# dalek-cryptography/curve25519-dalek

Hardware: NVIDIA H100
Metric: Pippenger MSM points/sec (higher is better)
Workload: dtype exact integers: f64 limbs (radix 2^51, FP64 pipe) in the bucket kernel, u32 limbs (radix 2^25.5) elsewhere

## Files before the change

### curve25519_dalek_b200/csrc/msm.cu

```cuda
#include <algorithm>
#include <cstdio>
#include <utility>
#include <vector>

#include "../../include/dalek_b200.h"
#include "engine.h"
#include "ge64.cuh"
#include "warp4.cuh"
#include "warp4_f64.cuh"

static inline unsigned cdiv(size_t a, unsigned b) { return (unsigned)((a + b - 1) / b); }

int ws_reserve(dalek_b200_ctx *ctx, DevBuf &b, size_t bytes)
{
    if (bytes <= b.cap) return 0;
    if (b.p) { cudaFree(b.p); b.p = nullptr; b.cap = 0; }
    size_t want = bytes + bytes / 8 + 256;
    cudaError_t e = cudaMalloc(&b.p, want);
    if (e != cudaSuccess) { ctx->last_error = std::string("cudaMalloc: ") + cudaGetErrorString(e); return DALEK_E_NOMEM; }
    b.cap = want;
    return 0;
}

int pinned_reserve(dalek_b200_ctx *ctx, size_t bytes)
{
    if (bytes <= ctx->h_pinned_cap) return 0;
    if (ctx->h_pinned) cudaFreeHost(ctx->h_pinned);
    ctx->h_pinned = nullptr; ctx->h_pinned_cap = 0;
    cudaError_t e = cudaMallocHost(&ctx->h_pinned, bytes + 4096);
    if (e != cudaSuccess) { ctx->last_error = std::string("cudaMallocHost: ") + cudaGetErrorString(e); return DALEK_E_NOMEM; }
    ctx->h_pinned_cap = bytes + 4096;
    return 0;
}

template <int F64>
__global__ void __launch_bounds__(128, 3) k_prep_compressed(const uint4 *__restrict__ in, ge_niels_packed *__restrict__ out, size_t n,
                                  int *__restrict__ bad)
{
    size_t i = (size_t)blockIdx.x * blockDim.x + threadIdx.x;
    if (i >= n) return;
    uint4 a = in[2 * i], b = in[2 * i + 1];
    uint32_t s[8] = {a.x, a.y, a.z, a.w, b.x, b.y, b.z, b.w};
    fe x, y;
    uint32_t ok = ge_decompress_affine<F64>(x, y, s);
    if (!ok) { atomicOr(bad, 1); fe_0(x); fe_1(y); }
    ge_niels nl; ge_affine_to_niels(nl, x, y);
    ge_niels_packed p; ge_niels_pack(p, nl);
    uint4 *o = reinterpret_cast<uint4 *>(out + i);
#pragma unroll
    for (int k = 0; k < 6; k++) o[k] = make_uint4(p.w[4 * k], p.w[4 * k + 1], p.w[4 * k + 2], p.w[4 * k + 3]);
}

template <int F64>
__global__ void k_prep_ristretto(const uint32_t *__restrict__ in, ge_niels_packed *__restrict__ out, size_t n, int *__restrict__ bad)
{
    size_t i = (size_t)blockIdx.x * blockDim.x + threadIdx.x;
    if (i >= n) return;
    uint32_t enc[8];
#pragma unroll
    for (int k = 0; k < 8; k++) enc[k] = in[8 * i + k];
    ge_p3 P;
    if (!ristretto_decompress<F64>(P, enc)) { atomicOr(bad, 1); ge_p3_identity(P); }
    ge_niels nl; ge_affine_to_niels(nl, P.X, P.Y);
    ge_niels_packed pk; ge_niels_pack(pk, nl);
    out[i] = pk;
}

#define PREP_THREADS 256
#define PREP_PER_THREAD 4
#define PREP_GROUP (PREP_THREADS * PREP_PER_THREAD)
#define PREP_NW (PREP_THREADS / 32)

__device__ __forceinline__ void load_coord_f64(fe64 &h, const uint64_t *__restrict__ src)
{
    uint64_t l[5];
#pragma unroll
    for (int k = 0; k < 5; k++) l[k] = __ldg(src + k);
    fe t; fe_from_limbs51(t, l);
    fe64_from_fe_limbs(h, t);
}
__device__ __forceinline__ void store_coord(uint4 *o, const fe64 &v, uint32_t ok, uint32_t c)
{
    fe f;
    uint32_t w[8];
    fe64_to_fe(f, v); fe_tobytes_words(w, f);
#pragma unroll
    for (int q = 0; q < 8; q++) w[q] = ok ? w[q] : (q == 0 ? c : 0u);
    o[0] = make_uint4(w[0], w[1], w[2], w[3]);
    o[1] = make_uint4(w[4], w[5], w[6], w[7]);
}
__device__ __forceinline__ uint32_t load_z(fe64 &h, const uint64_t *__restrict__ in, size_t i)
{
    uint64_t l[5];
#pragma unroll
    for (int k = 0; k < 5; k++) l[k] = __ldg(in + 20 * i + 10 + k);
    fe t; fe_from_limbs51(t, l);
    fe64_from_fe_limbs(h, t);
    return 1u - (uint32_t)fe_iszero(t);
}
__device__ __forceinline__ void fe64_shfl_up(fe64 &o, const fe64 &f, int d)
{
#pragma unroll
    for (int k = 0; k < 5; k++) o.v[k] = __shfl_up_sync(0xffffffffu, f.v[k], d);
}
__device__ __forceinline__ void fe64_shfl_down(fe64 &o, const fe64 &f, int d)
{
#pragma unroll
    for (int k = 0; k < 5; k++) o.v[k] = __shfl_down_sync(0xffffffffu, f.v[k], d);
}
__device__ __forceinline__ void fe64_shfl_xor(fe64 &o, const fe64 &f, int m)
{
#pragma unroll
    for (int k = 0; k < 5; k++) o.v[k] = __shfl_xor_sync(0xffffffffu, f.v[k], m);
}
__device__ __forceinline__ void fe64_shfl_idx(fe64 &o, const fe64 &f, int src)
{
#pragma unroll
    for (int k = 0; k < 5; k++) o.v[k] = __shfl_sync(0xffffffffu, f.v[k], src);
}

__device__ __forceinline__ void warp_product(fe64 &p, const fe64 &x, int width)
{
    fe64 t;
    p = x;
#pragma unroll 1
    for (int m = width >> 1; m > 0; m >>= 1) { fe64_shfl_xor(t, p, m); fe64_mul(p, p, t); }
}

__device__ __forceinline__ void warp_other_products(const fe64 &x, fe64 &below, fe64 &above, fe64 &all)
{
    const uint32_t lane = threadIdx.x & 31;
    fe64 lo = x, hi = x, t;
#pragma unroll 1
    for (int d = 1; d < 32; d <<= 1) {
        fe64_shfl_up(t, lo, d);
        if (lane >= (uint32_t)d) fe64_mul(lo, lo, t);
        fe64_shfl_down(t, hi, d);
        if (lane + d < 32) fe64_mul(hi, hi, t);
    }
    fe64_shfl_idx(all, lo, 31);
    fe64_shfl_up(below, lo, 1); if (lane == 0) fe64_1(below);
    fe64_shfl_down(above, hi, 1); if (lane == 31) fe64_1(above);
}

template <bool INVERT>
__device__ __forceinline__ void block_inverse(fe64 &inv, const fe64 &acc, fe64 *s_warp, const fe64 *tot_inv)
{
    const uint32_t lane = threadIdx.x & 31, warp = threadIdx.x >> 5, nw = blockDim.x >> 5;
    fe64 below, above, all;
    warp_other_products(acc, below, above, all);
    if (lane == 0) s_warp[warp] = all;
    __syncthreads();
    if (warp == 0) {
        fe64 x, b, a, t;
        if (lane < nw) x = s_warp[lane]; else fe64_1(x);
        warp_other_products(x, b, a, all);
        if (INVERT) {
            fe q; fe64_to_fe(q, all); fe_invert(q, q); fe64_from_fe_limbs(t, q);
        } else {
            t = *tot_inv;
        }
        fe64_mul(t, t, b); fe64_mul(t, t, a);
        if (lane < nw) s_warp[lane] = t;
    }
    __syncthreads();
    fe64_mul(inv, s_warp[warp], below); fe64_mul(inv, inv, above);
}

__global__ void __launch_bounds__(PREP_THREADS, 2)
k_prep_zprod(const uint64_t *__restrict__ in, fe64 *__restrict__ prod, size_t n)
{
    __shared__ fe64 s_warp[PREP_NW];
    const uint32_t tid = threadIdx.x, lane = tid & 31, warp = tid >> 5;
    const size_t g0 = (size_t)blockIdx.x * PREP_GROUP + tid;
    fe64 z[PREP_PER_THREAD], acc, t;
    uint32_t ok[PREP_PER_THREAD];
#pragma unroll
    for (int k = 0; k < PREP_PER_THREAD; k++) {
        const size_t i = g0 + (size_t)k * PREP_THREADS;
        if (i < n) ok[k] = load_z(z[k], in, i); else { ok[k] = 0; fe64_1(z[k]); }
    }
    acc = z[0];
    if (!ok[0]) fe64_1(acc);
#pragma unroll
    for (int k = 1; k < PREP_PER_THREAD; k++) { fe64_mul(t, acc, z[k]); fe64_cmov(acc, t, ok[k]); }
    warp_product(t, acc, 32);
    if (lane == 0) s_warp[warp] = t;
    __syncthreads();
    if (warp == 0) {
        if (lane < PREP_NW) acc = s_warp[lane]; else fe64_1(acc);
        warp_product(t, acc, PREP_NW);
        if (lane == 0) prod[blockIdx.x] = t;
    }
}

__global__ void __launch_bounds__(PREP_THREADS)
k_prep_invert(fe64 *__restrict__ prod, fe64 *__restrict__ pre, uint32_t G)
{
    __shared__ fe64 s_warp[PREP_NW];
    const uint32_t per = (G + blockDim.x - 1) / blockDim.x, b = min(threadIdx.x * per, G), e = min(b + per, G);
    fe64 acc, inv, t;
    fe64_1(acc);
    for (uint32_t k = b; k < e; k++) { fe64_mul(acc, acc, prod[k]); pre[k] = acc; }
    block_inverse<true>(inv, acc, s_warp, nullptr);
    for (uint32_t k = e; k-- > b;) {
        const fe64 x = prod[k];
        if (k > b) fe64_mul(t, inv, pre[k - 1]); else t = inv;
        prod[k] = t;
        fe64_mul(inv, inv, x);
    }
}

__global__ void __launch_bounds__(PREP_THREADS, 2)
k_prep_finish(const uint64_t *__restrict__ in, const fe64 *__restrict__ ginv, ge_niels_packed *__restrict__ out, size_t n)
{
    __shared__ fe64 s_warp[PREP_NW];
    __shared__ fe64 s_pre[PREP_PER_THREAD - 1][PREP_THREADS];
    const uint32_t tid = threadIdx.x;
    const size_t g0 = (size_t)blockIdx.x * PREP_GROUP + tid;
    fe64 acc, inv;
    uint32_t nz = 0;
    fe64_1(acc);
#pragma unroll 1
    for (int k = 0; k < PREP_PER_THREAD; k++) {
        const size_t i = g0 + (size_t)k * PREP_THREADS;
        if (k > 0) s_pre[k - 1][tid] = acc;
        if (i < n) {
            fe64 z, t;
            const uint32_t ok = load_z(z, in, i);
            fe64_mul(t, acc, z); fe64_cmov(acc, t, ok);
            nz |= ok << k;
        }
    }
    block_inverse<false>(inv, acc, s_warp, ginv + blockIdx.x);
#pragma unroll 1
    for (int k = PREP_PER_THREAD - 1; k >= 0; k--) {
        const size_t i = g0 + (size_t)k * PREP_THREADS;
        if (i >= n) continue;
        const uint32_t ok = (nz >> k) & 1u;
        const uint64_t *src = in + 20 * i;
        fe64 X, Y, zi, u, v;
        load_coord_f64(u, src + 10);
        if (k > 0) fe64_mul(zi, inv, s_pre[k - 1][tid]); else zi = inv;
        fe64_mul(v, inv, u); fe64_cmov(inv, v, ok);
        uint4 *o = reinterpret_cast<uint4 *>(out + i);
        load_coord_f64(X, src); load_coord_f64(Y, src + 5);
        fe64_add(u, Y, X); fe64_mul(v, u, zi);
        store_coord(o, v, ok, 1u);
        fe64_sub(u, Y, X); fe64_mul(v, u, zi);
        store_coord(o + 2, v, ok, 1u);
        load_coord_f64(u, src + 15);
        fe64_mul(v, u, zi); fe64_const_2d(u); fe64_mul(v, v, u);
        store_coord(o + 4, v, ok, 0u);
    }
}

__global__ void k_prep_extended_pniels(const uint64_t *__restrict__ in, ge_pniels_packed *__restrict__ out, size_t n)
{
    size_t i = (size_t)blockIdx.x * blockDim.x + threadIdx.x;
    if (i >= n) return;
    const ulonglong2 *src = reinterpret_cast<const ulonglong2 *>(in + 20 * i);
    uint64_t l[20];
#pragma unroll
    for (int k = 0; k < 10; k++) { ulonglong2 v = src[k]; l[2 * k] = v.x; l[2 * k + 1] = v.y; }
    ge_p3 p;
    fe_from_limbs51(p.X, l); fe_from_limbs51(p.Y, l + 5); fe_from_limbs51(p.Z, l + 10); fe_from_limbs51(p.T, l + 15);
    ge_pniels pn; ge_p3_to_pniels(pn, p);
    ge_pniels_packed pk; ge_pniels_pack(pk, pn);
    uint4 *o = reinterpret_cast<uint4 *>(out + i);
#pragma unroll
    for (int k = 0; k < 8; k++) o[k] = make_uint4(pk.w[4 * k], pk.w[4 * k + 1], pk.w[4 * k + 2], pk.w[4 * k + 3]);
}

int msm_prepared_kind(int point_fmt, int kind)
{
    return point_fmt == DALEK_POINTS_EXTENDED ? kind : PK_NIELS;
}

int msm_prepare_points_on(dalek_b200_ctx *ctx, cudaStream_t st, const void *d_in, int point_fmt, size_t n, void *d_out, int *d_bad,
                          int kind)
{
    if (n == 0) return 0;
    if (point_fmt == DALEK_POINTS_COMPRESSED) {
        if (ctx->opt_decompress_f64) k_prep_compressed<1><<<cdiv(n, 128), 128, 0, st>>>((const uint4 *)d_in, (ge_niels_packed *)d_out, n, d_bad);
        else k_prep_compressed<0><<<cdiv(n, 128), 128, 0, st>>>((const uint4 *)d_in, (ge_niels_packed *)d_out, n, d_bad);
    } else if (point_fmt == DALEK_POINTS_RISTRETTO) {
        if (ctx->opt_decompress_f64) k_prep_ristretto<1><<<cdiv(n, 128), 128, 0, st>>>((const uint32_t *)d_in, (ge_niels_packed *)d_out, n, d_bad);
        else k_prep_ristretto<0><<<cdiv(n, 128), 128, 0, st>>>((const uint32_t *)d_in, (ge_niels_packed *)d_out, n, d_bad);
    } else if (kind == PK_PNIELS) {
        k_prep_extended_pniels<<<cdiv(n, 128), 128, 0, st>>>((const uint64_t *)d_in, (ge_pniels_packed *)d_out, n);
    } else {
        const unsigned G = cdiv(n, PREP_GROUP);
        int rc;
        if ((rc = ws_reserve(ctx, ctx->prep_prod, 2 * (size_t)G * sizeof(fe64)))) return rc;
        fe64 *prod = (fe64 *)ctx->prep_prod.p;
        k_prep_zprod<<<G, PREP_THREADS, 0, st>>>((const uint64_t *)d_in, prod, n);
        k_prep_invert<<<1, PREP_THREADS, 0, st>>>(prod, prod + G, G);
        k_prep_finish<<<G, PREP_THREADS, 0, st>>>((const uint64_t *)d_in, prod, (ge_niels_packed *)d_out, n);
        ctx->launches += 2;
    }
    ctx->launches++;
    CUDA_TRY(ctx, cudaGetLastError());
    return 0;
}

int msm_prepare_points(dalek_b200_ctx *ctx, const void *d_in, int point_fmt, size_t n, void *d_out, int *d_bad, int kind)
{
    return msm_prepare_points_on(ctx, ctx->stream, d_in, point_fmt, n, d_out, d_bad, kind);
}

int msm_window_count_for_bits(int c) { return 256 / c + 1; }
// ... 474 lines not shown
    ge_p3 acc;
    if (F64) {
        ge64_p3 acc64;
        if (fold_old) {
            ge_p3 old; load_p3(old, buckets + t);
            fe64_from_fe(acc64.X, old.X); fe64_from_fe(acc64.Y, old.Y); fe64_from_fe(acc64.Z, old.Z); fe64_from_fe(acc64.T, old.T);
        } else {
            ge64_identity(acc64);
        }
        uint32_t e_next = len ? idx[0] : 0;
        if (TMA) {
            const uint32_t bar0 = (uint32_t)__cvta_generic_to_shared(&s_bar[0][threadIdx.x]);
            const uint32_t bar1 = (uint32_t)__cvta_generic_to_shared(&s_bar[1][threadIdx.x]);
            asm volatile("mbarrier.init.shared::cta.b64 [%0], 1;" ::"r"(bar0) : "memory");
            asm volatile("mbarrier.init.shared::cta.b64 [%0], 1;" ::"r"(bar1) : "memory");
            asm volatile("fence.mbarrier_init.release.cluster;" ::: "memory");
            asm volatile("fence.proxy.async.shared::cta;" ::: "memory");
        }
        auto prefetch = [&](uint32_t e, int buf) {
            const uint32_t pi = e & 0x7fffffffu;
            const char *src = reinterpret_cast<const char *>(points) + (size_t)pi * (NQ * 16);
            if (TMA) {
                const uint32_t bar = (uint32_t)__cvta_generic_to_shared(&s_bar[buf][threadIdx.x]);
                const uint32_t dst = (uint32_t)__cvta_generic_to_shared(&s_bulk[buf][threadIdx.x][0]);
                asm volatile("mbarrier.arrive.expect_tx.shared::cta.b64 _, [%0], %1;" ::"r"(bar), "r"(NQ * 16) : "memory");
                asm volatile("cp.async.bulk.shared::cluster.global.mbarrier::complete_tx::bytes [%0], [%1], %2, [%3];"
                             ::"r"(dst), "l"(src), "r"(NQ * 16), "r"(bar) : "memory");
            } else {
#pragma unroll
                for (int q = 0; q < NQ; q++) {
                    uint32_t dst = (uint32_t)__cvta_generic_to_shared(&s_pts[buf][q][threadIdx.x]);
                    asm volatile("cp.async.cg.shared.global [%0], [%1], 16;" ::"r"(dst), "l"(src + 16 * q) : "memory");
                }
            }
        };
        if (len) prefetch(e_next, 0);
        if (!TMA) asm volatile("cp.async.commit_group;" ::: "memory");
        for (uint32_t k = 0; k < len; k++) {
            const uint32_t e = e_next, neg = e >> 31;
            const int buf = k & 1;
            if (k + 1 < len) { e_next = idx[k + 1]; prefetch(e_next, buf ^ 1); }
            uint32_t words[NQ * 4];
            if (TMA) {
                const uint32_t bar = (uint32_t)__cvta_generic_to_shared(&s_bar[buf][threadIdx.x]);
                const uint32_t parity = (k >> 1) & 1u;
                uint32_t done;
                do {
                    asm volatile("{ .reg .pred p; mbarrier.try_wait.parity.shared::cta.b64 p, [%1], %2; selp.u32 %0, 1, 0, p; }"
                                 : "=r"(done) : "r"(bar), "r"(parity) : "memory");
                } while (!done);
                const uint4 *sp = reinterpret_cast<const uint4 *>(&s_bulk[buf][threadIdx.x][0]);
#pragma unroll
                for (int q = 0; q < NQ; q++) { uint4 v = sp[q]; words[4 * q] = v.x; words[4 * q + 1] = v.y; words[4 * q + 2] = v.z; words[4 * q + 3] = v.w; }
            } else {
                asm volatile("cp.async.commit_group;" ::: "memory");
                asm volatile("cp.async.wait_group 1;" ::: "memory");
#pragma unroll
                for (int q = 0; q < NQ; q++) { uint4 v = s_pts[buf][q][threadIdx.x]; words[4 * q] = v.x; words[4 * q + 1] = v.y; words[4 * q + 2] = v.z; words[4 * q + 3] = v.w; }
            }
            ge_niels_packed pk;
#pragma unroll
            for (int q = 0; q < 24; q++) pk.w[q] = words[q];
            ge64_niels nl; ge64_niels_unpack(nl, pk);
            ge64_madd(acc64, acc64, nl, neg);
        }
        ge64_to_p3(acc, acc64);
    } else {
    if (fold_old) load_p3(acc, buckets + t); else ge_p3_identity(acc);
    for (uint32_t k = 0; k < len; k++) {
        uint32_t e = idx[k];
        uint32_t neg = e >> 31, pi = e & 0x7fffffffu;
        const uint4 *src = reinterpret_cast<const uint4 *>(reinterpret_cast<const ge_niels_packed *>(points) + pi);
        ge_niels_packed pk;
#pragma unroll
        for (int q = 0; q < 6; q++) { uint4 v = __ldg(src + q); pk.w[4 * q] = v.x; pk.w[4 * q + 1] = v.y; pk.w[4 * q + 2] = v.z; pk.w[4 * q + 3] = v.w; }
        ge_niels nl; ge_niels_unpack(nl, pk);
        ge_madd(acc, acc, nl, neg);
    }
    }
    ge_p3_raw r; ge_p3_store_raw(r, acc);
    uint4 *o = reinterpret_cast<uint4 *>(!split ? buckets + t : task_sums + p);
#pragma unroll
    for (int q = 0; q < 10; q++) o[q] = make_uint4(r.w[4 * q], r.w[4 * q + 1], r.w[4 * q + 2], r.w[4 * q + 3]);
}


__global__ void __launch_bounds__(128)
k_heavy_fixup(const uint32_t *__restrict__ heavy, const uint32_t *__restrict__ ntasks, const uint32_t *__restrict__ task_off,
              const uint32_t *__restrict__ win_base, uint32_t nbuckets, uint32_t w0, uint32_t w1,
              const ge_p3_raw *__restrict__ task_sums, ge_p3_raw *__restrict__ buckets, int first)
{
    const uint32_t lane = threadIdx.x & 31, role = lane & 3, grp = lane >> 2;
    const uint32_t nwarps = (gridDim.x * blockDim.x) >> 5;
    const uint32_t nheavy = heavy[0];
    for (uint32_t h = (blockIdx.x * blockDim.x + threadIdx.x) >> 5; h < nheavy; h += nwarps) {
        uint32_t tb = heavy[1 + h];
        if (tb / nbuckets < w0 || tb / nbuckets >= w1) continue;
        uint32_t kk = ntasks[tb];
        uint32_t base = win_base[tb / nbuckets] + task_off[tb];
        w4_point acc, x;
        if (first || grp != 0) w4_identity(acc); else w4_load(acc, buckets + tb);
        for (uint32_t j0 = 0; j0 < kk; j0 += 8) {
            uint32_t j = j0 + grp;
            if (j < kk) w4_load(x, task_sums + base + j); else w4_identity(x);
            w4_add(acc, x, role);
        }
        for (int d = 16; d >= 4; d >>= 1) { w4_shfl_down(x, acc, d); w4_add(acc, x, role); }
        if (grp == 0) w4_store(buckets + tb, acc, role);
    }
}

__device__ __forceinline__ void load_p3_f64(ge64_p3 &o, const ge_p3_raw *src)
{
    ge_p3 q; load_p3(q, src);
    fe64_from_fe_limbs(o.X, q.X); fe64_from_fe_limbs(o.Y, q.Y); fe64_from_fe_limbs(o.Z, q.Z); fe64_from_fe_limbs(o.T, q.T);
}

__global__ void __launch_bounds__(32)
k_chunk_reduce_f64(const ge_p3_raw *__restrict__ S_in, uint32_t n_in, uint32_t m, uint32_t n_out, uint32_t nwin,
                   ge_p3_raw *__restrict__ S_out, ge_p3_raw *__restrict__ W_out)
{
    const uint32_t t = blockIdx.x * blockDim.x + threadIdx.x;
    if (t >= n_out * nwin) return;
    const uint32_t w = t / n_out, q = t % n_out;
    const ge_p3_raw *S = S_in + (size_t)w * n_in + (size_t)q * m;
    fe64 d2; fe64_const_2d(d2);
    ge64_p3 run, acc, x;
    load_p3_f64(run, S + (m - 1));
    acc = run;
    ge_p3 nxt;
    if (m > 1) load_p3(nxt, S + (m - 2));
#pragma unroll 1
    for (uint32_t r = m - 1; r-- > 0;) {
        fe64_from_fe_limbs(x.X, nxt.X); fe64_from_fe_limbs(x.Y, nxt.Y); fe64_from_fe_limbs(x.Z, nxt.Z); fe64_from_fe_limbs(x.T, nxt.T);
        if (r > 0) load_p3(nxt, S + (r - 1));
        ge64_add_p3(run, run, x, d2);
        ge64_add_p3(acc, acc, run, d2);
    }
    ge_p3 o; ge_p3_raw raw;
    ge64_to_p3(o, run); ge_p3_store_raw(raw, o);
    uint4 *d = reinterpret_cast<uint4 *>(S_out + t);
#pragma unroll
    for (int k = 0; k < 10; k++) d[k] = make_uint4(raw.w[4 * k], raw.w[4 * k + 1], raw.w[4 * k + 2], raw.w[4 * k + 3]);
    ge64_to_p3(o, acc); ge_p3_store_raw(raw, o);
    d = reinterpret_cast<uint4 *>(W_out + t);
#pragma unroll
    for (int k = 0; k < 10; k++) d[k] = make_uint4(raw.w[4 * k], raw.w[4 * k + 1], raw.w[4 * k + 2], raw.w[4 * k + 3]);
}

__global__ void __launch_bounds__(128)
k_chunk_reduce(const ge_p3_raw *__restrict__ S_in, uint32_t n_in, uint32_t m, uint32_t one_based, uint32_t n_out,
               uint32_t nwin, ge_p3_raw *__restrict__ S_out, ge_p3_raw *__restrict__ W_out)
{
    const uint32_t role = threadIdx.x & 3;
    const uint32_t total = n_out * nwin;
    uint32_t t = (blockIdx.x * blockDim.x + threadIdx.x) >> 2;
    if (((blockIdx.x * blockDim.x + (threadIdx.x & ~31u)) >> 2) >= total) return;
    const bool live = t < total;
    if (!live) t = total - 1;
    const uint32_t w = t / n_out, q = t % n_out;
    const ge_p3_raw *S = S_in + (size_t)w * n_in + (size_t)q * m;
    w4_point run, acc, x;
    w4_load(run, S + (m - 1));
    acc = run;
    for (uint32_t r = m - 1; r-- > 1;) {
        w4_load(x, S + r);
        w4_add(run, x, role);
        w4_add(acc, run, role);
    }
    if (m > 1) {
        w4_load(x, S);
        w4_add(run, x, role);
        if (one_based) w4_add(acc, run, role);
    } else if (!one_based) {
        w4_identity(acc);
    }
    if (live) { w4_store(S_out + t, run, role); w4_store(W_out + t, acc, role); }
}

#define SUM_PIECE 256u
__global__ void __launch_bounds__(128)
k_plain_sum(const ge_p3_raw *__restrict__ pool, const uint2 *__restrict__ desc, ge_p3_raw *__restrict__ out)
{
    __shared__ ge_p3_raw sh[32];
    const uint32_t role = threadIdx.x & 3, grp = threadIdx.x >> 2;
    const uint2 d = desc[blockIdx.x];
    const ge_p3_raw *a = pool + d.x;
    const uint32_t len = d.y;
    w4_point acc, x;
    w4_identity(acc);
    for (uint32_t i0 = 0; i0 < len; i0 += 32) {
        uint32_t i = i0 + grp;
        if (i < len) w4_load(x, a + i); else w4_identity(x);
        w4_add(acc, x, role);
    }
    w4_store(&sh[grp], acc, role);
    __syncthreads();
    for (uint32_t d = 16; d > 0; d >>= 1) {
        if (threadIdx.x < 32 * ((d + 7) / 8)) {
            uint32_t g2 = grp < d ? grp + d : grp;
            w4_load(acc, &sh[grp]); w4_load(x, &sh[g2]);
            w4_add(acc, x, role);
        }
        __syncthreads();
        if (grp < d) w4_store(&sh[grp], acc, role);
        __syncthreads();
    }
    if (grp == 0) { w4_load(acc, &sh[0]); w4_store(out + blockIdx.x, acc, role); }
}

struct LevelInfo { int nlevels; int log2m[16]; };
__global__ void __launch_bounds__(128)
k_finish_windows(const ge_p3_raw *__restrict__ S_top, const ge_p3_raw *__restrict__ A, LevelInfo li, uint32_t nwin,
                 ge_p3_raw *__restrict__ out)
{
    const uint32_t role = threadIdx.x & 3;
    uint32_t w = (blockIdx.x * blockDim.x + threadIdx.x) >> 2;
    if (((blockIdx.x * blockDim.x + (threadIdx.x & ~31u)) >> 2) >= nwin) return;
    const bool live = w < nwin;
    if (!live) w = nwin - 1;
    w4_point t, x;
    if (li.nlevels > 0) {
        w4_load(t, A + (size_t)(li.nlevels - 1) * nwin + w);
        for (int l = li.nlevels - 2; l >= 0; l--) {
            for (int k = 0; k < li.log2m[l]; k++) w4_dbl(t, role, k == li.log2m[l] - 1);
            w4_load(x, A + (size_t)l * nwin + w);
            w4_add(t, x, role);
        }
    } else {
        w4_load(t, S_top + w);
    }
    if (live) w4_store(out + w, t, role);
}

__global__ void __launch_bounds__(32)
k_combine(const ge_p3_raw *__restrict__ windows, int ranks, int nwin, int c, MsmResult *__restrict__ res)
{
    const uint32_t role = threadIdx.x & 3;
    w4f_point tot;
    w4f_horner(tot, windows, ranks, nwin, c, role);
    if (threadIdx.x != 0) return;
    ge_p3 total; w4f_to_p3(total, tot);
    uint32_t s[8];
    ge_compress(s, total);
#pragma unroll
    for (int i = 0; i < 8; i++) res->compressed[i] = s[i];
    fe_to_limbs51(res->limbs, total.X); fe_to_limbs51(res->limbs + 5, total.Y);
    fe_to_limbs51(res->limbs + 10, total.Z); fe_to_limbs51(res->limbs + 15, total.T);
    res->is_identity = ge_is_identity(total);
    res->pad = 0;
}

static int msm_sort_fine_bits(size_t entries_per_window, int c, int hist_windows)
{
    int lg = std::max(0, c - 1 - SORT_FINE_MAX);
    while (lg < c - 1 && ((size_t)SORT_BIN_MEAN << lg) < entries_per_window && (2u << lg) <= SORT_NC_MAX &&
           ((size_t)hist_windows << (lg + 1)) <= SORT_HIST_MAX)
        lg++;
    return c - 1 - lg;
}

int msm_accumulate_chunk(dalek_b200_ctx *ctx, const uint32_t *d_scalars, const ge_niels_packed *d_points, size_t n,
                         int c, bool first, int active_windows, size_t flat, cudaEvent_t points_ready)
{
    const int nwin_d = msm_window_count_for_bits(c);
    const int nact = active_windows > 0 && active_windows < nwin_d ? active_windows : nwin_d;
    const int nwin = flat ? 1 : nwin_d;
    const uint32_t nb = 1u << (c - 1);
    const size_t total_buckets = (size_t)nwin * nb;
    const uint32_t task_len = flat ? msm_task_len(n * (size_t)nact, 1, nb) : msm_task_len(n, nact, nb);
    const size_t max_tasks = total_buckets + (std::max<size_t>(1, n) * nact) / task_len + 1;
    const size_t max_heavy = (std::max<size_t>(1, n) * nact) / task_len + 1;
    const uint32_t parts = (nb + SCAN_PART - 1) / SCAN_PART;
    const int F = msm_sort_fine_bits(flat ? n * (size_t)nact : n, c, flat ? 1 : nact);
    const uint32_t nc = nb >> F;
    cudaStream_t st = ctx->stream;
    int rc;
    if ((rc = ws_reserve(ctx, ctx->counts, (total_buckets + (size_t)nwin * nc + 1 + max_heavy) * 4))) return rc;
    if ((rc = ws_reserve(ctx, ctx->offsets, (total_buckets + (size_t)nwin * parts + 2 * (size_t)nwin * nc + nwin) * 4))) return rc;
    if ((rc = ws_reserve(ctx, ctx->ntasks, total_buckets * 4))) return rc;
    if ((rc = ws_reserve(ctx, ctx->task_off, total_buckets * 4 + (nwin + 1) * 4))) return rc;
    if ((rc = ws_reserve(ctx, ctx->tasks, max_tasks * 8))) return rc;
    if ((rc = ws_reserve(ctx, ctx->task_sums, max_tasks * sizeof(ge_p3_raw)))) return rc;
    if ((rc = ws_reserve(ctx, ctx->task_order, (3 * TASK_BINS + max_tasks) * 4))) return rc;
    if ((rc = ws_reserve(ctx, ctx->digits, std::max<size_t>(1, n) * nact * 8))) return rc;
    if ((rc = ws_reserve(ctx, ctx->sorted, std::max<size_t>(1, n) * nact * 4))) return rc;
    if ((rc = ws_reserve(ctx, ctx->buckets, total_buckets * sizeof(ge_p3_raw)))) return rc;
    uint32_t *counts = (uint32_t *)ctx->counts.p, *offsets = (uint32_t *)ctx->offsets.p;
    uint32_t *ntasks = (uint32_t *)ctx->ntasks.p, *task_off = (uint32_t *)ctx->task_off.p;
    uint32_t *win_base = task_off + total_buckets;
    uint32_t *ccount = counts + total_buckets, *heavy = ccount + (size_t)nwin * nc;
    uint32_t *part_sums = offsets + total_buckets, *ccursor = part_sums + (size_t)nwin * parts;
    uint32_t *xpre = ccursor + (size_t)nwin * nc, *xtot = xpre + (size_t)nwin * nc;
    uint2 *tasks = (uint2 *)ctx->tasks.p;
    uint32_t *t_hist = (uint32_t *)ctx->task_order.p, *t_cursor = t_hist + TASK_BINS, *t_start = t_cursor + TASK_BINS;
    uint32_t *order = t_start + TASK_BINS;
    ge_p3_raw *task_sums = (ge_p3_raw *)ctx->task_sums.p;
    uint2 *records = (uint2 *)ctx->digits.p;
    uint32_t *sorted = (uint32_t *)ctx->sorted.p;
    ge_p3_raw *buckets = (ge_p3_raw *)ctx->buckets.p;

    const size_t part_smem = SORT_TILE * 8 + (2 * (size_t)nc + 33) * 4;
    const size_t fine_smem = SORT_FINE_CAP * 12 + ((1u << F) + 33) * 4;
    CUDA_TRY(ctx, cudaFuncSetAttribute(k_sort_partition, cudaFuncAttributeMaxDynamicSharedMemorySize, (int)part_smem));
    CUDA_TRY(ctx, cudaFuncSetAttribute(k_sort_fine, cudaFuncAttributeMaxDynamicSharedMemorySize, (int)fine_smem));
    CUDA_TRY(ctx, cudaMemsetAsync(ccount, 0, ((size_t)nwin * nc + 1) * 4, st));
    CUDA_TRY(ctx, cudaMemsetAsync(t_hist, 0, 2 * TASK_BINS * 4, st));
    if (n) {
        k_sort_count<<<cdiv(n, SORT_COUNT_TILE), SORT_THREADS, 0, st>>>((const uint4 *)d_scalars, n, c, nact, F, nc, flat ? 1 : 0, ccount);
        ctx->launches++;
    }
    k_sort_bins_scan<<<nwin, SORT_THREADS, 0, st>>>(ccount, nc, F, nb, ccursor, xpre, xtot, counts, ntasks);
    if (n) {
        k_sort_partition<<<cdiv(n, SORT_TILE), SORT_THREADS, part_smem, st>>>((const uint4 *)d_scalars, n, c, nact, F, nc, nb, flat,
                                                                              ccount, ccursor, records, counts);
        ctx->launches++;
    }
    const size_t extra = n * (size_t)nact / SORT_FINE_CAP;
    k_sort_fine<<<(unsigned)(nwin * nc + extra), SORT_THREADS, fine_smem, st>>>(records, ccount, ccursor, xpre, xtot, n, F, nc, nb,
                                                                               (uint32_t)nwin, flat ? 1 : 0, counts, offsets, sorted, ntasks);
    k_task_count<<<cdiv(total_buckets, 256), 256, 0, st>>>(counts, (uint32_t)total_buckets, task_len, ntasks, heavy);
    k_scan_partial<<<nwin * parts, 1024, 0, st>>>(ntasks, nb, parts, part_sums);
    k_scan_bases<<<nwin, 32, 0, st>>>(part_sums, parts);
    k_scan_apply<<<nwin * parts, 1024, 0, st>>>(ntasks, part_sums, nb, parts, task_off);
    k_task_bases<<<1, 32, 0, st>>>(ntasks, task_off, nb, nwin, win_base);
    k_task_fill<<<cdiv(total_buckets, 256), 256, 0, st>>>(ntasks, task_off, win_base, nb, (uint32_t)total_buckets, tasks);
    k_task_hist<<<cdiv(max_tasks, 256), 256, 0, st>>>(tasks, counts, win_base + nwin, task_len, t_hist);
    k_task_scan<<<1, 256, 0, st>>>(t_hist, t_start);
    k_task_scatter<<<cdiv(max_tasks, 256), 256, 0, st>>>(tasks, counts, win_base + nwin, task_len, t_start, t_cursor, order);
    ctx->launches += 11;
    if (points_ready) CUDA_TRY(ctx, cudaStreamWaitEvent(st, points_ready, 0));
    if (first) CUDA_TRY(ctx, cudaEventRecord(ctx->ev_a, st));
    {
        const unsigned grid = cdiv(max_tasks, 128);
        const int f = first ? 1 : 0;
#define LAUNCH_ACC(F64_, TMA_) k_bucket_accumulate<F64_, TMA_><<<grid, 128, 0, st>>>(d_points, sorted, counts, offsets, ntasks, tasks, order, win_base, 0, nwin, n, nb, task_len, buckets, task_sums, f)
        const bool tma = ctx->opt_field_f64 && ctx->opt_acc_tma;
        if (tma) LAUNCH_ACC(1, 1); else if (ctx->opt_field_f64) LAUNCH_ACC(1, 0); else LAUNCH_ACC(0, 0);
#undef LAUNCH_ACC
        k_heavy_fixup<<<ctx->sm_count * 4, 128, 0, st>>>(heavy, ntasks, task_off, win_base, nb, 0u, (uint32_t)nwin, task_sums, buckets, f);
        ctx->launches += 2;
    }
    CUDA_TRY(ctx, cudaEventRecord(ctx->ev_b, st));
    ctx->last_kernel_launches = first ? 1 : ctx->last_kernel_launches + 1;
    CUDA_TRY(ctx, cudaGetLastError());
    return 0;
}

int msm_reduce_finish(dalek_b200_ctx *ctx, int c, ge_p3_raw *d_windows, MsmResult *d_result, bool flat)
{
    const int nwin = flat ? 1 : msm_window_count_for_bits(c);
    const int desc_key = c + (flat ? 64 : 0);
    const uint32_t nb = 1u << (c - 1);
    cudaStream_t st = ctx->stream;
    int rc;
    ge_p3_raw *buckets = (ge_p3_raw *)ctx->buckets.p;
    LevelInfo li; li.nlevels = 0;
    std::vector<uint32_t> lvl_m, lvl_nout;
    size_t pool_pts = 0;
    {
        uint32_t n_in = nb; bool first = true;
        while (n_in > 1) {
            uint32_t m = first ? std::min<uint32_t>(n_in, 16) : std::min<uint32_t>(n_in, 8);
            uint32_t n_out = (n_in + m - 1) / m;
            lvl_m.push_back(m); lvl_nout.push_back(n_out);
            int lg = 0; while ((1u << lg) < m) lg++;
            li.log2m[li.nlevels++] = lg;
            pool_pts += 2 * (size_t)n_out * nwin;
            n_in = n_out; first = false;
        }
    }
    if ((rc = ws_reserve(ctx, ctx->red_a, std::max<size_t>(1, pool_pts) * sizeof(ge_p3_raw)))) return rc;
    if ((rc = ws_reserve(ctx, ctx->red_b, (size_t)16 * nwin * sizeof(ge_p3_raw)))) return rc;
    ge_p3_raw *pool = (ge_p3_raw *)ctx->red_a.p, *A = (ge_p3_raw *)ctx->red_b.p;
    const ge_p3_raw *S_in = buckets;
    uint32_t n_in = nb;
    size_t pos = 0;
    std::vector<std::pair<size_t, uint32_t>> w_arrays;
    for (int l = 0; l < li.nlevels; l++) {
        uint32_t m = lvl_m[l], n_out = lvl_nout[l];
        ge_p3_raw *S_out = pool + pos, *W_out = pool + pos + (size_t)n_out * nwin;
        if (l == 0 && ctx->opt_field_f64 && n_in % m == 0)
            k_chunk_reduce_f64<<<cdiv((size_t)n_out * nwin, 32), 32, 0, st>>>(S_in, n_in, m, n_out, nwin, S_out, W_out);
        else
            k_chunk_reduce<<<cdiv((size_t)n_out * nwin * 4, 128), 128, 0, st>>>(S_in, n_in, m, l == 0 ? 1u : 0u, n_out, nwin, S_out, W_out);
        ctx->launches++;
        w_arrays.push_back({pos + (size_t)n_out * nwin, n_out});
        S_in = S_out; n_in = n_out; pos += 2 * (size_t)n_out * nwin;
    }
    {
        std::vector<uint2> d1, d2;
        for (int l = 0; l < li.nlevels; l++)
            for (int w = 0; w < nwin; w++) {
                uint32_t off = (uint32_t)(w_arrays[l].first + (size_t)w * w_arrays[l].second), len = w_arrays[l].second;
                uint32_t first_piece = (uint32_t)d1.size();
                for (uint32_t o = 0; o < len; o += SUM_PIECE) d1.push_back(make_uint2(off + o, std::min(SUM_PIECE, len - o)));
                d2.push_back(make_uint2(first_piece, (uint32_t)d1.size() - first_piece));
            }
        const size_t n1 = d1.size(), n2 = d2.size();
        if ((rc = ws_reserve(ctx, ctx->sum_desc, (n1 + n2) * sizeof(uint2)))) return rc;
        if ((rc = ws_reserve(ctx, ctx->sum_part, n1 * sizeof(ge_p3_raw)))) return rc;
        uint2 *dd1 = (uint2 *)ctx->sum_desc.p, *dd2 = dd1 + n1;
        if (ctx->sum_desc_c != desc_key) {
            CUDA_TRY(ctx, cudaMemcpyAsync(dd1, d1.data(), n1 * sizeof(uint2), cudaMemcpyHostToDevice, st));
            CUDA_TRY(ctx, cudaMemcpyAsync(dd2, d2.data(), n2 * sizeof(uint2), cudaMemcpyHostToDevice, st));
            CUDA_TRY(ctx, cudaStreamSynchronize(st));
            ctx->sum_desc_c = desc_key;
        }
        ge_p3_raw *parts = (ge_p3_raw *)ctx->sum_part.p;
        k_plain_sum<<<(unsigned)n1, 128, 0, st>>>(pool, dd1, parts);
        k_plain_sum<<<(unsigned)n2, 128, 0, st>>>(parts, dd2, A);
        ctx->launches += 2;
    }
    k_finish_windows<<<cdiv((size_t)nwin * 4, 128), 128, 0, st>>>(S_in, A, li, nwin, d_windows);
    ctx->launches++;
    if (d_result) {
        k_combine<<<1, 32, 0, st>>>(d_windows, 1, nwin, c, d_result);
        ctx->launches++;
    }
    CUDA_TRY(ctx, cudaGetLastError());
    return 0;
}

int msm_combine_windows(dalek_b200_ctx *ctx, const ge_p3_raw *d_windows, int ranks, int nwin, int c, MsmResult *d_result)
{
    k_combine<<<1, 32, 0, ctx->stream>>>(d_windows, ranks, nwin, c, d_result);
    ctx->launches++;
    CUDA_TRY(ctx, cudaGetLastError());
    return 0;
}
```

### curve25519_dalek_b200/csrc/warp4_f64.cuh

```cuda
#pragma once
#include "ge64.cuh"

#if defined(__CUDACC__)
#define W4_DEV __device__ __forceinline__
W4_DEV uint32_t w4_lane() { return threadIdx.x & 31u; }
W4_DEV uint32_t w4_shfl(uint32_t v, int src) { return __shfl_sync(0xffffffffu, v, src); }
W4_DEV uint32_t w4_shfl_down(uint32_t v, int delta) { return __shfl_down_sync(0xffffffffu, v, delta); }
W4_DEV bool w4_any(bool p) { return __any_sync(0xffffffffu, p) != 0; }
W4_DEV long long w4_bits(double d) { return __double_as_longlong(d); }
W4_DEV double w4_from_bits(long long b) { return __longlong_as_double(b); }
#else
#include <string.h>
#define W4_DEV static inline
uint32_t w4_lane();
uint32_t w4_shfl(uint32_t v, int src);
uint32_t w4_shfl_down(uint32_t v, int delta);
bool w4_any(bool p);
W4_DEV long long w4_bits(double d) { long long b; memcpy(&b, &d, 8); return b; }
W4_DEV double w4_from_bits(long long b) { double d; memcpy(&d, &b, 8); return d; }
#endif

struct w4f_point { fe64 X, Y, Z, T; };

W4_DEV void fe64_sel4(fe64 &o, const fe64 &a0, const fe64 &a1, const fe64 &a2, const fe64 &a3, uint32_t role)
// ... 60 lines not shown
    fe64_sub(E, S2, Yp);
    fe64_add(F, ZZ, ZZ); fe64_sub(F, F, Ym);
    fe64_carry(F, F);
    fe64_sel4(f, E, Yp, Ym, E, role);
    fe64_sel4(g, F, Ym, F, Yp, role);
    fe64_mul(r, f, g);
    fe64_gbcast(p.X, r, 0); fe64_gbcast(p.Y, r, 1); fe64_gbcast(p.Z, r, 2);
    if (want_t) fe64_gbcast(p.T, r, 3);
}

W4_DEV void w4f_add_tail(w4f_point &p, const fe64 &a, const fe64 &b, const fe64 &c, const fe64 &D, uint32_t neg, uint32_t role)
{
    fe64 E, H, DpC, DmC, F, G, f, g, r;
    fe64_sub(E, b, a); fe64_add(H, b, a);
    fe64_add(DpC, D, c); fe64_sub(DmC, D, c);
    fe64_carry(DmC, DmC);
    F = DmC; fe64_cmov(F, DpC, neg);
    G = DpC; fe64_cmov(G, DmC, neg);
    fe64_sel4(f, F, G, DmC, E, role);
    fe64_sel4(g, E, H, DpC, H, role);
    fe64_mul(r, f, g);
    fe64_gbcast(p.X, r, 0); fe64_gbcast(p.Y, r, 1); fe64_gbcast(p.Z, r, 2); fe64_gbcast(p.T, r, 3);
}

W4_DEV void w4f_add(w4f_point &p, const w4f_point &q, const fe64 &d2, uint32_t role)
{
    fe64 qYpX, qYmX, qT2d, A, B, f, g, r, a, b, c, zz, D;
    fe64_add(qYpX, q.Y, q.X);
    fe64_sub(qYmX, q.Y, q.X);
    fe64_sub(A, p.Y, p.X); fe64_add(B, p.Y, p.X);
    fe64_mul(qT2d, q.T, d2);
    fe64_sel4(f, A, B, p.T, p.Z, role);
    fe64_sel4(g, qYmX, qYpX, qT2d, q.Z, role);
    fe64_mul(r, f, g);
    fe64_gbcast(a, r, 0); fe64_gbcast(b, r, 1); fe64_gbcast(c, r, 2); fe64_gbcast(zz, r, 3);
    fe64_add(D, zz, zz);
    w4f_add_tail(p, a, b, c, D, 0u, role);
}

W4_DEV void w4f_padd(w4f_point &p, const ge_pniels_packed &pk, uint32_t neg, uint32_t role)
{
    ge64_pniels q; ge64_pniels_unpack(q, pk);
    fe64 qp = q.YpX, qm = q.YmX;
    { fe64 t = qp; fe64_cmov(qp, qm, neg); fe64_cmov(qm, t, neg); }
    fe64 A, B, f, g, r, a, b, c, zz, D;
    fe64_sub(A, p.Y, p.X); fe64_add(B, p.Y, p.X);
    fe64_sel4(f, A, B, p.T, p.Z, role);
    fe64_sel4(g, qm, qp, q.T2d, q.Z, role);
    fe64_mul(r, f, g);
    fe64_gbcast(a, r, 0); fe64_gbcast(b, r, 1); fe64_gbcast(c, r, 2); fe64_gbcast(zz, r, 3);
    fe64_add(D, zz, zz);
    w4f_add_tail(p, a, b, c, D, neg, role);
}

W4_DEV void w4f_shfl_down(w4f_point &o, const w4f_point &p, int delta_lanes)
{
    const fe64 *src[4] = {&p.X, &p.Y, &p.Z, &p.T};
    fe64 *dst[4] = {&o.X, &o.Y, &o.Z, &o.T};
#pragma unroll
    for (int c = 0; c < 4; c++)
#pragma unroll
        for (int k = 0; k < 5; k++) {
            const long long v = w4_bits(src[c]->v[k]);
            const uint32_t lo = w4_shfl_down((uint32_t)v, delta_lanes), hi = w4_shfl_down((uint32_t)(v >> 32), delta_lanes);
            dst[c]->v[k] = w4_from_bits((long long)(((uint64_t)hi << 32) | lo));
        }
}

W4_DEV void w4f_to_p3(ge_p3 &o, const w4f_point &p)
{
    fe64_to_fe(o.X, p.X); fe64_to_fe(o.Y, p.Y); fe64_to_fe(o.Z, p.Z); fe64_to_fe(o.T, p.T);
}

FE_HD void fe64_const_2d(fe64 &d2) { fe k; fe_const_2d(k); fe64_from_fe_limbs(d2, k); }

struct w20_role { uint32_t g, i, base; };
W4_DEV w20_role w20_roles() { const uint32_t l = w4_lane(); w20_role r; r.g = (l / 5u) & 3u; r.i = l % 5u; r.base = 5u * r.g; return r; }

W4_DEV double w20_shfl(double v, uint32_t src)
{
    const long long b = w4_bits(v);
    const uint32_t lo = w4_shfl((uint32_t)b, (int)src), hi = w4_shfl((uint32_t)((uint64_t)b >> 32), (int)src);
    return w4_from_bits((long long)(((uint64_t)hi << 32) | lo));
}
W4_DEV long long w20_shfl_ll(long long b, uint32_t src)
{
    const uint32_t lo = w4_shfl((uint32_t)b, (int)src), hi = w4_shfl((uint32_t)((uint64_t)b >> 32), (int)src);
    return (long long)(((uint64_t)hi << 32) | lo);
}

W4_DEV double w20_carry(double f, const w20_role &r)
{
#if FE64_DEV
    const double C = 6755399441055744.0;
    const double q = __fma_rn(f, 1.0 / 2251799813685248.0, C) - C;
    const double rr = __fma_rn(q, -2251799813685248.0, f);
#else
    const double q = nearbyint(f / 2251799813685248.0), rr = f - q * 2251799813685248.0;
#endif
    const double qp = w20_shfl(q, r.base + (r.i + 4u) % 5u);
    return rr + (r.i == 0 ? 19.0 * qp : qp);
}

W4_DEV void w20_split(long long &f, long long &lo, double a, double b, double b_scaled )
{
#if FE64_DEV
    const double M1 = 6755399441055744.0;
    const double K = 6755399441055744.0 * 4503599627370496.0 + 4503599627370496.0;
    const double t = __fma_rz(a, b_scaled, M1);
    const double u = __fma_rn(t, -4503599627370496.0, K);
    const double l = __fma_rn(a, b, u);
    f = __double_as_longlong(t) - (FE64_E52 + (1LL << 51));
    lo = __double_as_longlong(l) - FE64_E52;
#else
    (void)b_scaled;
    const __int128 p = (__int128)(long long)a * (__int128)(long long)b, lim = (__int128)1 << 103;
    assert(p < lim && p > -lim);
    f = (long long)(p >> 52);
    lo = (long long)(p - ((__int128)f << 52));
#endif
}

W4_DEV double w20_mul(double a_own, double b_own, const w20_role &r)
{
    double b[5];
#pragma unroll
    for (uint32_t j = 0; j < 5; j++) b[j] = w20_shfl(b_own, r.base + j);
    long long f[5], lo[5];
#pragma unroll
    for (int d = 0; d < 5; d++) w20_split(f[d], lo[d], a_own, b[d], b[d] * (1.0 / 4503599627370496.0));
    long long U[5];
    U[0] = lo[0] + 38 * f[4];
#pragma unroll
    for (uint32_t e = 1; e < 5; e++) {
        const long long v = lo[e] + 2 * f[e - 1];
        U[e] = r.i + e >= 5u ? 19 * v : v;
    }
    long long R = U[0];
#pragma unroll
    for (uint32_t d = 1; d < 5; d++) R += w20_shfl_ll(U[d], r.base + (r.i + 5u - d) % 5u);
    const long long q = (R + (1LL << 50)) >> 51;
    const long long rr = R - q * (1LL << 51);
    long long qp = (long long)(int32_t)w4_shfl((uint32_t)(int32_t)q, (int)(r.base + (r.i + 4u) % 5u));
    if (r.i == 0) qp *= 19;
    const long long limb = rr + qp;
#if FE64_DEV
    return __longlong_as_double((limb + (1LL << 51)) | FE64_E52) - (FE64_TWO52 + FE64_TWO51);
#else
    assert(limb < (1LL << 50) + (1LL << 15) && limb > -(1LL << 50) - (1LL << 15));
    return (double)limb;
#endif
}

W4_DEV double w20_take(const w4f_point &p, const w20_role &r)
{
    double v = 0.0;
#pragma unroll
    for (uint32_t k = 0; k < 5; k++) {
        const double x = r.g == 0 ? p.X.v[k] : r.g == 1 ? p.Y.v[k] : r.g == 2 ? p.Z.v[k] : p.T.v[k];
        if (r.i == k) v = x;
    }
    return v;
}
W4_DEV void w20_give(w4f_point &p, double c)
{
#pragma unroll
    for (uint32_t k = 0; k < 5; k++) {
        p.X.v[k] = w20_shfl(c, k); p.Y.v[k] = w20_shfl(c, 5u + k); p.Z.v[k] = w20_shfl(c, 10u + k); p.T.v[k] = w20_shfl(c, 15u + k);
    }
}

W4_DEV void w20_dbl(double &c, const w20_role &r)
{
    const double x = w20_shfl(c, r.i), y = w20_shfl(c, 5u + r.i);
    const double s = w20_carry(x + y, r);
    const double in = r.g == 3 ? s : c;
    const double sq = w20_mul(in, in, r);
    const double xx = w20_shfl(sq, r.i), yy = w20_shfl(sq, 5u + r.i), zz = w20_shfl(sq, 10u + r.i), s2 = w20_shfl(sq, 15u + r.i);
    const double Yp = yy + xx, Ym = yy - xx;
    const double E = s2 - Yp;
    const double F = w20_carry(zz + zz - Ym, r);
    const double a = r.g == 1 ? Yp : r.g == 2 ? Ym : E;
    const double b = r.g == 1 ? Ym : r.g == 3 ? Yp : F;
    c = w20_mul(a, b, r);
}

W4_DEV void w20_dbl_n(w4f_point &p, int k)
{
    const w20_role r = w20_roles();
    double c = w20_take(p, r);
#if FE64_DEV
#pragma unroll 1
#endif
    for (int t = 0; t < k; t++) w20_dbl(c, r);
    w20_give(p, c);
}

W4_DEV void w4f_horner(w4f_point &tot, const ge_p3_raw *windows, int ranks, int nwin, int c, uint32_t role)
{
    fe64 d2; fe64_const_2d(d2);
    w4f_point x;
    w4f_identity(tot);
    bool started = false;
#pragma unroll 1
    for (int w = nwin - 1; w >= 0; w--) {
        if (started) {
            w20_dbl_n(tot, c);
        } else {
            bool any = false;
#pragma unroll 1
            for (int r = 0; r < ranks; r++) {
                ge_p3 q; ge_p3_raw raw;
#if defined(__CUDA_ARCH__)
                const uint4 *s4 = reinterpret_cast<const uint4 *>(windows + (size_t)r * nwin + w);
#pragma unroll
                for (int k = 0; k < 10; k++) { uint4 v = s4[k]; raw.w[4 * k] = v.x; raw.w[4 * k + 1] = v.y; raw.w[4 * k + 2] = v.z; raw.w[4 * k + 3] = v.w; }
#else
                raw = windows[(size_t)r * nwin + w];
#endif
                ge_p3_load_raw(q, raw);
                any |= !ge_is_identity(q);
            }
            if (!any) continue;
            started = true;
        }
#pragma unroll 1
        for (int r = 0; r < ranks; r++) { w4f_load(x, windows + (size_t)r * nwin + w); w4f_add(tot, x, d2, role); }
    }
}
```

Baseline: 359.6 million.

## Port reduction, finish, combine and inversion to 20-lane f64 warp arithmetic

Moves the chunk-reduce, finish-windows and combine kernels from a 4-lane u32 point representation to a 20-lane-per-point f64 scheme, where each lane holds one limb of one coordinate. Field inversion in the block-inverse prep and in the final encoding now runs as a warp-parallel f64 addition chain instead of a single-thread u32 invert. The aim is to use the FP64 pipe and more lanes per point in these latency-bound tail stages. In exchange, only one point is processed per warp instead of eight, so these kernels have far fewer points in flight and rely on many more shuffles.

New measurement: 372.8 million (median of 6 runs). 1.04x the previous value.

```diff
diff --git a/curve25519_dalek_b200/csrc/msm.cu b/curve25519_dalek_b200/csrc/msm.cu
--- a/curve25519_dalek_b200/csrc/msm.cu
+++ b/curve25519_dalek_b200/csrc/msm.cu
@@ -156,7 +156,10 @@
         if (lane < nw) x = s_warp[lane]; else fe64_1(x);
         warp_other_products(x, b, a, all);
         if (INVERT) {
-            fe q; fe64_to_fe(q, all); fe_invert(q, q); fe64_from_fe_limbs(t, q);
+            const w20_role r = w20_roles();
+            const double inv = w20_invert(w20_limb(all, r.i), r);
+#pragma unroll
+            for (uint32_t k = 0; k < 5; k++) t.v[k] = w20_shfl(inv, k);
         } else {
             t = *tot_inv;
         }
@@ -937,30 +940,26 @@
 k_chunk_reduce(const ge_p3_raw *__restrict__ S_in, uint32_t n_in, uint32_t m, uint32_t one_based, uint32_t n_out,
                uint32_t nwin, ge_p3_raw *__restrict__ S_out, ge_p3_raw *__restrict__ W_out)
 {
-    const uint32_t role = threadIdx.x & 3;
-    const uint32_t total = n_out * nwin;
-    uint32_t t = (blockIdx.x * blockDim.x + threadIdx.x) >> 2;
-    if (((blockIdx.x * blockDim.x + (threadIdx.x & ~31u)) >> 2) >= total) return;
-    const bool live = t < total;
-    if (!live) t = total - 1;
+    const uint32_t t = (blockIdx.x * blockDim.x + threadIdx.x) >> 5;
+    if (t >= n_out * nwin) return;
+    const w20_role rl = w20_roles();
+    const double d2 = w20_const_2d(rl);
     const uint32_t w = t / n_out, q = t % n_out;
     const ge_p3_raw *S = S_in + (size_t)w * n_in + (size_t)q * m;
-    w4_point run, acc, x;
-    w4_load(run, S + (m - 1));
-    acc = run;
+    double run = w20_load(S + (m - 1), rl), acc = run;
+#pragma unroll 1
     for (uint32_t r = m - 1; r-- > 1;) {
-        w4_load(x, S + r);
-        w4_add(run, x, role);
-        w4_add(acc, run, role);
+        w20_add(run, w20_load(S + r, rl), d2, rl);
+        w20_add(acc, run, d2, rl);
     }
     if (m > 1) {
-        w4_load(x, S);
-        w4_add(run, x, role);
-        if (one_based) w4_add(acc, run, role);
+        w20_add(run, w20_load(S, rl), d2, rl);
+        if (one_based) w20_add(acc, run, d2, rl);
     } else if (!one_based) {
-        w4_identity(acc);
-    }
-    if (live) { w4_store(S_out + t, run, role); w4_store(W_out + t, acc, role); }
+        acc = w20_identity(rl);
+    }
+    w20_store(S_out + t, run);
+    w20_store(W_out + t, acc);
 }
 
 #define SUM_PIECE 256u
@@ -999,35 +998,33 @@
 k_finish_windows(const ge_p3_raw *__restrict__ S_top, const ge_p3_raw *__restrict__ A, LevelInfo li, uint32_t nwin,
                  ge_p3_raw *__restrict__ out)
 {
-    const uint32_t role = threadIdx.x & 3;
-    uint32_t w = (blockIdx.x * blockDim.x + threadIdx.x) >> 2;
-    if (((blockIdx.x * blockDim.x + (threadIdx.x & ~31u)) >> 2) >= nwin) return;
-    const bool live = w < nwin;
-    if (!live) w = nwin - 1;
-    w4_point t, x;
+    const uint32_t w = (blockIdx.x * blockDim.x + threadIdx.x) >> 5;
+    if (w >= nwin) return;
+    const w20_role rl = w20_roles();
+    double t;
     if (li.nlevels > 0) {
-        w4_load(t, A + (size_t)(li.nlevels - 1) * nwin + w);
+        const double d2 = w20_const_2d(rl);
+        t = w20_load(A + (size_t)(li.nlevels - 1) * nwin + w, rl);
+#pragma unroll 1
         for (int l = li.nlevels - 2; l >= 0; l--) {
-            for (int k = 0; k < li.log2m[l]; k++) w4_dbl(t, role, k == li.log2m[l] - 1);
-            w4_load(x, A + (size_t)l * nwin + w);
-            w4_add(t, x, role);
+#pragma unroll 1
+            for (int k = 0; k < li.log2m[l]; k++) w20_dbl(t, rl);
+            w20_add(t, w20_load(A + (size_t)l * nwin + w, rl), d2, rl);
         }
     } else {
-        w4_load(t, S_top + w);
-    }
-    if (live) w4_store(out + w, t, role);
+        t = w20_load(S_top + w, rl);
+    }
+    w20_store(out + w, t);
 }
 
 __global__ void __launch_bounds__(32)
 k_combine(const ge_p3_raw *__restrict__ windows, int ranks, int nwin, int c, MsmResult *__restrict__ res)
 {
-    const uint32_t role = threadIdx.x & 3;
-    w4f_point tot;
-    w4f_horner(tot, windows, ranks, nwin, c, role);
+    const w20_role r = w20_roles();
+    uint32_t s[8];
+    ge_p3 total;
+    w20_encode(s, total, w20_horner(windows, ranks, nwin, c, r), r);
     if (threadIdx.x != 0) return;
-    ge_p3 total; w4f_to_p3(total, tot);
-    uint32_t s[8];
-    ge_compress(s, total);
 #pragma unroll
     for (int i = 0; i < 8; i++) res->compressed[i] = s[i];
     fe_to_limbs51(res->limbs, total.X); fe_to_limbs51(res->limbs + 5, total.Y);
@@ -1168,7 +1165,7 @@
         if (l == 0 && ctx->opt_field_f64 && n_in % m == 0)
             k_chunk_reduce_f64<<<cdiv((size_t)n_out * nwin, 32), 32, 0, st>>>(S_in, n_in, m, n_out, nwin, S_out, W_out);
         else
-            k_chunk_reduce<<<cdiv((size_t)n_out * nwin * 4, 128), 128, 0, st>>>(S_in, n_in, m, l == 0 ? 1u : 0u, n_out, nwin, S_out, W_out);
+            k_chunk_reduce<<<cdiv((size_t)n_out * nwin * 32, 128), 128, 0, st>>>(S_in, n_in, m, l == 0 ? 1u : 0u, n_out, nwin, S_out, W_out);
         ctx->launches++;
         w_arrays.push_back({pos + (size_t)n_out * nwin, n_out});
         S_in = S_out; n_in = n_out; pos += 2 * (size_t)n_out * nwin;
@@ -1197,7 +1194,7 @@
         k_plain_sum<<<(unsigned)n2, 128, 0, st>>>(parts, dd2, A);
         ctx->launches += 2;
     }
-    k_finish_windows<<<cdiv((size_t)nwin * 4, 128), 128, 0, st>>>(S_in, A, li, nwin, d_windows);
+    k_finish_windows<<<cdiv((size_t)nwin * 32, 128), 128, 0, st>>>(S_in, A, li, nwin, d_windows);
     ctx->launches++;
     if (d_result) {
         k_combine<<<1, 32, 0, st>>>(d_windows, 1, nwin, c, d_result);
diff --git a/curve25519_dalek_b200/csrc/warp4_f64.cuh b/curve25519_dalek_b200/csrc/warp4_f64.cuh
--- a/curve25519_dalek_b200/csrc/warp4_f64.cuh
+++ b/curve25519_dalek_b200/csrc/warp4_f64.cuh
@@ -236,6 +236,41 @@
 #endif
 }
 
+W4_DEV double w20_sq(double a, const w20_role &r) { return w20_mul(a, a, r); }
+
+W4_DEV double w20_sqn(double a, int n, const w20_role &r)
+{
+#if FE64_DEV
+#pragma unroll 1
+#endif
+    for (int k = 0; k < n; k++) a = w20_sq(a, r);
+    return a;
+}
+
+W4_DEV double w20_invert(double z, const w20_role &r)
+{
+    const double t0 = w20_sq(z, r);
+    const double t2 = w20_mul(z, w20_sqn(t0, 2, r), r);
+    const double t3 = w20_mul(t0, t2, r);
+    const double t5 = w20_mul(t2, w20_sq(t3, r), r);
+    const double t7 = w20_mul(w20_sqn(t5, 5, r), t5, r);
+    const double t9 = w20_mul(w20_sqn(t7, 10, r), t7, r);
+    const double t11 = w20_mul(w20_sqn(t9, 20, r), t9, r);
+    const double t13 = w20_mul(w20_sqn(t11, 10, r), t7, r);
+    const double t15 = w20_mul(w20_sqn(t13, 50, r), t13, r);
+    const double t17 = w20_mul(w20_sqn(t15, 100, r), t15, r);
+    const double t19 = w20_mul(w20_sqn(t17, 50, r), t13, r);
+    return w20_mul(w20_sqn(t19, 5, r), t3, r);
+}
+
+W4_DEV double w20_limb(const fe64 &a, uint32_t i)
+{
+    double v = 0.0;
+#pragma unroll
+    for (uint32_t k = 0; k < 5; k++) if (i == k) v = a.v[k];
+    return v;
+}
+
 W4_DEV double w20_take(const w4f_point &p, const w20_role &r)
 {
     double v = 0.0;
@@ -280,16 +315,67 @@
     w20_give(p, c);
 }
 
-W4_DEV void w4f_horner(w4f_point &tot, const ge_p3_raw *windows, int ranks, int nwin, int c, uint32_t role)
-{
-    fe64 d2; fe64_const_2d(d2);
-    w4f_point x;
-    w4f_identity(tot);
+W4_DEV void w20_add(double &c, double q, double d2, const w20_role &r)
+{
+    const double qT2d = w20_mul(w20_shfl(q, 15u + r.i), d2, r);
+    const double qx = w20_shfl(q, r.i), qy = w20_shfl(q, 5u + r.i);
+    const double x = w20_shfl(c, r.i), y = w20_shfl(c, 5u + r.i);
+    const double f = r.g == 0 ? y - x : r.g == 1 ? y + x : c;
+    const double g = r.g == 0 ? qy - qx : r.g == 1 ? qy + qx : r.g == 2 ? q : qT2d;
+    const double m = w20_mul(f, g, r);
+    const double a = w20_shfl(m, r.i), b = w20_shfl(m, 5u + r.i), zz = w20_shfl(m, 10u + r.i), cc = w20_shfl(m, 15u + r.i);
+    const double D = zz + zz;
+    const double E = b - a, H = b + a;
+    const double DpC = D + cc;
+    const double DmC = w20_carry(D - cc, r);
+    const double f2 = r.g == 1 ? DpC : r.g == 3 ? E : DmC;
+    const double g2 = r.g == 0 ? E : r.g == 2 ? DpC : H;
+    c = w20_mul(f2, g2, r);
+}
+
+W4_DEV double w20_load(const ge_p3_raw *src, const w20_role &r)
+{
+    const uint32_t *w = src->w + 10u * r.g + 2u * r.i;
+    const uint64_t l = (uint64_t)w[0] + ((uint64_t)w[1] << 26);
+#if FE64_DEV
+    const double t = __longlong_as_double((long long)l | FE64_E52) - FE64_TWO52;
+#else
+    const double t = (double)l;
+#endif
+    return w20_carry(t, r);
+}
+
+W4_DEV void w20_store(ge_p3_raw *dst, double c)
+{
+    const uint32_t g = w4_lane() & 3u;
+    fe64 v;
+#pragma unroll
+    for (uint32_t k = 0; k < 5; k++) v.v[k] = w20_shfl(c, 5u * g + k);
+    if (w4_lane() >= 4u) return;
+    fe o; fe64_to_fe(o, v);
+    uint32_t *d = dst->w + 10u * g;
+#if defined(__CUDA_ARCH__)
+#pragma unroll
+    for (int k = 0; k < 10; k += 2) *reinterpret_cast<uint2 *>(d + k) = make_uint2(o.v[k], o.v[k + 1]);
+#else
+    for (int k = 0; k < 10; k++) d[k] = o.v[k];
+#endif
+}
+
+W4_DEV double w20_const_2d(const w20_role &r) { fe64 d2; fe64_const_2d(d2); return w20_limb(d2, r.i); }
+
+W4_DEV double w20_identity(const w20_role &r) { return (r.g == 1 || r.g == 2) && r.i == 0 ? 1.0 : 0.0; }
+
+W4_DEV double w20_horner(const ge_p3_raw *windows, int ranks, int nwin, int c, const w20_role &rl)
+{
+    const double d2 = w20_const_2d(rl);
+    double tot = w20_identity(rl);
     bool started = false;
 #pragma unroll 1
     for (int w = nwin - 1; w >= 0; w--) {
         if (started) {
-            w20_dbl_n(tot, c);
+#pragma unroll 1
+            for (int t = 0; t < c; t++) w20_dbl(tot, rl);
         } else {
             bool any = false;
 #pragma unroll 1
@@ -309,6 +395,26 @@
             started = true;
         }
 #pragma unroll 1
-        for (int r = 0; r < ranks; r++) { w4f_load(x, windows + (size_t)r * nwin + w); w4f_add(tot, x, d2, role); }
-    }
-}
+        for (int r = 0; r < ranks; r++) w20_add(tot, w20_load(windows + (size_t)r * nwin + w, rl), d2, rl);
+    }
+    return tot;
+}
+
+W4_DEV void w4f_horner(w4f_point &tot, const ge_p3_raw *windows, int ranks, int nwin, int c, uint32_t )
+{
+    w20_give(tot, w20_horner(windows, ranks, nwin, c, w20_roles()));
+}
+
+W4_DEV void w20_encode(uint32_t s[8], ge_p3 &P, double c, const w20_role &r)
+{
+    const double zinv = w20_invert(w20_shfl(c, 10u + r.i), r);
+    const double aff = w20_mul(c, zinv, r);
+    w4f_point p; w20_give(p, c);
+    fe64 x64, y64;
+#pragma unroll
+    for (uint32_t k = 0; k < 5; k++) { x64.v[k] = w20_shfl(aff, k); y64.v[k] = w20_shfl(aff, 5u + k); }
+    w4f_to_p3(P, p);
+    fe x, y; fe64_to_fe(x, x64); fe64_to_fe(y, y64);
+    fe_tobytes_words(s, y);
+    s[7] ^= (uint32_t)fe_isnegative(x) << 31;
+}
```
